# PierfrancescoArdino/C2M

Measured on AMD Instinct MI355X. Metric: generator train-step frames/sec at 128x256x7, higher is better.
Workload: dtype f32; 1 GPU; BASELINE configs[1]: 128x256, 7-frame clips (2 in + 5 predicted), batch 8/GPU, fp32, generator fwd+bwd only (no D), VGG loss on, random-init weights; global_batch=8, parallelism=single

## Files before the change

### c2m_amd/csrc/norm.hip

```cpp
#include "common.h"
#include "dtype.h"
#include <stdlib.h>

#define NORM_CHUNK 8192

struct NormShape { int N, C; long S; int mode; int chunks; };

static inline int norm_chunks(long S) { return (int)((S + NORM_CHUNK - 1) / NORM_CHUNK); }

template <class T>
__global__ __launch_bounds__(256) void norm_partial_kernel(const T* __restrict__ x, float* __restrict__ partial,
                                                            long S, int chunks) {
    __shared__ float sm[4];
    const long plane = blockIdx.x / chunks;
    const int chunk = blockIdx.x % chunks;
    const long beg = (long)chunk * NORM_CHUNK;
    const long end = beg + NORM_CHUNK < S ? beg + NORM_CHUNK : S;
    const T* __restrict__ p = x + plane * S;
    const int cnt = (int)(end - beg);
    const bool vec = (S & 3) == 0 && c2m_aligned(C2mVec4<T>::mask + 1, x);
    float s = 0.f;
    constexpr int NV = NORM_CHUNK / 1024;
    float4 keep[NV];
    if (vec) {
#pragma unroll
        for (int k = 0; k < NV; ++k) {
            const long i = beg + threadIdx.x * 4 + (long)k * 1024;
            if (i < end) {
                keep[k] = c2m_ld4(p + i);
                s += (keep[k].x + keep[k].y) + (keep[k].z + keep[k].w);
            }
        }
    } else {
        for (long i = beg + threadIdx.x; i < end; i += 256) s += c2m_ld(p, i);
    }
    s = block_sum_256(s, sm);
    const float mean = s / (float)cnt;
    float m2 = 0.f;
    if (vec) {
#pragma unroll
        for (int k = 0; k < NV; ++k) {
            const long i = beg + threadIdx.x * 4 + (long)k * 1024;
            if (i < end) {
                const float a = keep[k].x - mean, b = keep[k].y - mean, c = keep[k].z - mean, d = keep[k].w - mean;
                m2 += (a * a + b * b) + (c * c + d * d);
            }
        }
    } else {
        for (long i = beg + threadIdx.x; i < end; i += 256) { const float d = c2m_ld(p, i) - mean; m2 += d * d; }
    }
    m2 = block_sum_256(m2, sm);
    if (threadIdx.x == 0) {
        partial[(long)blockIdx.x * 2 + 0] = mean;
        partial[(long)blockIdx.x * 2 + 1] = m2;
    }
}

__global__ void norm_finalize_kernel(const float* __restrict__ partial, float* __restrict__ mean_out,
                                     float* __restrict__ invstd_out, float* __restrict__ running_mean,
                                     float* __restrict__ running_var, NormShape sh, float eps, float momentum) {
    const int nstat = sh.mode == 0 ? sh.N * sh.C : sh.C;
    const int i = blockIdx.x * blockDim.x + threadIdx.x;
    if (i >= nstat) return;
    double n = 0.0, mean = 0.0, m2 = 0.0;
    const int nrep = sh.mode == 0 ? 1 : sh.N;
    for (int r = 0; r < nrep; ++r) {
        const long plane = sh.mode == 0 ? i : (long)r * sh.C + i;
        for (int c = 0; c < sh.chunks; ++c) {
            const long beg = (long)c * NORM_CHUNK;
            const double nb = (double)((beg + NORM_CHUNK < sh.S ? beg + NORM_CHUNK : sh.S) - beg);
            const double mb = partial[(plane * sh.chunks + c) * 2 + 0];
            const double vb = partial[(plane * sh.chunks + c) * 2 + 1];
            const double tot = n + nb;
            const double delta = mb - mean;
            mean += delta * nb / tot;
            m2 += vb + delta * delta * n * nb / tot;
            n = tot;
        }
    }
    const double var = m2 / n;
    mean_out[i] = (float)mean;
    invstd_out[i] = (float)(1.0 / sqrt(var + (double)eps));
    if (running_mean) {
        const double unbiased = n > 1.0 ? m2 / (n - 1.0) : var;
        running_mean[i] = (float)((1.0 - momentum) * running_mean[i] + momentum * mean);
        running_var[i] = (float)((1.0 - momentum) * running_var[i] + momentum * unbiased);
    }
}

__global__ __launch_bounds__(256) void norm_finalize_bn_kernel(const float* __restrict__ partial,
                                                               float* __restrict__ mean_out,
                                                               float* __restrict__ invstd_out,
                                                               float* __restrict__ running_mean,
                                                               float* __restrict__ running_var, NormShape sh, float eps,
                                                               float momentum) {
    const int lane = threadIdx.x & 63;
    const int ch = blockIdx.x * 4 + (threadIdx.x >> 6);
    if (ch >= sh.C) return;
    double n = 0.0, mean = 0.0, m2 = 0.0;
    const int total = sh.N * sh.chunks;
    for (int e = lane; e < total; e += 64) {
        const int r = e / sh.chunks, c = e - r * sh.chunks;
        const long q = (((long)r * sh.C + ch) * sh.chunks + c) * 2;
        const long beg = (long)c * NORM_CHUNK;
        const double nb = (double)((beg + NORM_CHUNK < sh.S ? beg + NORM_CHUNK : sh.S) - beg);
        const double mb = partial[q], vb = partial[q + 1];
        const double tot = n + nb, delta = mb - mean;
        mean += delta * nb / tot;
        m2 += vb + delta * delta * n * nb / tot;
        n = tot;
    }
#pragma unroll
    for (int o = 32; o > 0; o >>= 1) {
        const double nb = __shfl_down(n, o, 64), mb = __shfl_down(mean, o, 64), vb = __shfl_down(m2, o, 64);
        const double tot = n + nb;
        if (tot > 0.0) {
            const double delta = mb - mean;
            mean += delta * nb / tot;
            m2 += vb + delta * delta * n * nb / tot;
            n = tot;
        }
    }
    if (lane != 0) return;
    const double var = m2 / n;
    mean_out[ch] = (float)mean;
    invstd_out[ch] = (float)(1.0 / sqrt(var + (double)eps));
    if (running_mean) {
        const double unbiased = n > 1.0 ? m2 / (n - 1.0) : var;
        running_mean[ch] = (float)((1.0 - momentum) * running_mean[ch] + momentum * mean);
        running_var[ch] = (float)((1.0 - momentum) * running_var[ch] + momentum * unbiased);
    }
}

C2M_API long c2m_norm_workspace_floats(int N, int C, long S) { return (long)N * C * norm_chunks(S) * 4; }

C2M_API int c2m_norm_stats(const void* x, float* mean, float* invstd, float* running_mean, float* running_var,
                           float* workspace, int N, int C, long S, int mode, float eps, float momentum, int dt, void* stream) {
    C2M_ENTER();
    if ((long)N * C * S <= 0) return 0;
    NormShape sh{N, C, S, mode, norm_chunks(S)};
    hipStream_t s = (hipStream_t)stream;
    C2M_DISPATCH_DT(dt, hipLaunchKernelGGL(norm_partial_kernel<T>, dim3((unsigned)((long)N * C * sh.chunks)), dim3(256), 0, s,
                                           (const T*)x, workspace, S, sh.chunks););
    const int nstat = mode == 0 ? N * C : C;
    if (mode == 1 && N * sh.chunks >= 16)
        hipLaunchKernelGGL(norm_finalize_bn_kernel, dim3(c2m_cdiv(C, 4)), dim3(256), 0, s, workspace, mean, invstd,
                           running_mean, running_var, sh, eps, momentum);
    else
        hipLaunchKernelGGL(norm_finalize_kernel, dim3(c2m_cdiv(nstat, 128)), dim3(128), 0, s, workspace, mean, invstd,
                           running_mean, running_var, sh, eps, momentum);
    return (int)hipGetLastError();
}

template <class T>
struct ApplyP {
    const T* x; const float* mean; const float* invstd; const float* gamma; const float* beta; const T* gb;
    T* y;
    int N, C; long S; int mode; int act; float slope;
};

template <class T>
__global__ void norm_apply_kernel(const ApplyP<T> p) {
    const long total = (long)p.N * p.C * p.S;
    for (long i = blockIdx.x * (long)blockDim.x + threadIdx.x; i < total; i += (long)gridDim.x * blockDim.x) {
        const long plane = i / p.S;
        const long s = i - plane * p.S;
        const int c = (int)(plane % p.C);
        const int n = (int)(plane / p.C);
        const int st = p.mode == 0 ? (int)plane : c;
        const float xhat = (c2m_ld(p.x, i) - p.mean[st]) * p.invstd[st];
        float v;
        if (p.gb) {
            const long gbase = ((long)n * 2 * p.C + c) * p.S + s;
            v = xhat * (1.0f + c2m_ld(p.gb, gbase)) + c2m_ld(p.gb, gbase + (long)p.C * p.S);
        } else if (p.gamma) {
            v = xhat * p.gamma[c] + p.beta[c];
        } else {
            v = xhat;
        }
        c2m_st(p.y, i, c2m_act(v, p.act, p.slope));
    }
}

template <class T>
// ... 158 lines not shown
    }
    m2 = block_sum_256(m2, sm);
    const double var = (double)m2 / (double)S;
    const float invstd = (float)(1.0 / sqrt(var + (double)eps));
    if (threadIdx.x == 0) { mean_out[plane] = mean; invstd_out[plane] = invstd; }
    const float ga = p.gamma ? p.gamma[c] : 1.f, be = p.gamma ? p.beta[c] : 0.f;
    T* __restrict__ y = p.y + plane * p.S;
    const T* __restrict__ g0 = p.gb ? p.gb + ((long)n * 2 * p.C + c) * p.S : nullptr;
    const T* __restrict__ g1 = p.gb ? g0 + (long)p.C * p.S : nullptr;
#pragma unroll
    for (int k = 0; k < NV; ++k) {
        const int i = threadIdx.x * 4 + k * 1024;
        if (i < S) {
            const float4 v = keep[k];
            float4 sc = make_float4(ga, ga, ga, ga), sh = make_float4(be, be, be, be);
            if (p.gb) {
                const float4 a = c2m_ld4(g0 + i);
                sc = make_float4(1.0f + a.x, 1.0f + a.y, 1.0f + a.z, 1.0f + a.w);
                sh = c2m_ld4(g1 + i);
            }
            float4 o;
            o.x = c2m_act((v.x - mean) * invstd * sc.x + sh.x, p.act, p.slope);
            o.y = c2m_act((v.y - mean) * invstd * sc.y + sh.y, p.act, p.slope);
            o.z = c2m_act((v.z - mean) * invstd * sc.z + sh.z, p.act, p.slope);
            o.w = c2m_act((v.w - mean) * invstd * sc.w + sh.w, p.act, p.slope);
            c2m_st4(y + i, o);
        }
    }
}

template <class T, int NE>
__global__ __launch_bounds__(256) void norm_bn_small_fused_kernel(const ApplyP<T> p, float* __restrict__ mean_out,
                                                                  float* __restrict__ invstd_out, float* __restrict__ running_mean,
                                                                  float* __restrict__ running_var, float eps, float momentum) {
    __shared__ float sm[4];
    const int c = blockIdx.x;
    const int S = (int)p.S, total = p.N * S;
    const long cstride = (long)p.C * p.S;
    const unsigned magic = (unsigned)((0x100000000ULL + (unsigned)S - 1) / (unsigned)S);
    const T* __restrict__ xc = p.x + (long)c * p.S;
    float keep[NE];
    float s = 0.f;
#pragma unroll
    for (int k = 0; k < NE; ++k) {
        const int e = threadIdx.x + k * 256;
        keep[k] = 0.f;
        if (e < total) {
            const int n = S == 1 ? e : (int)__umulhi((unsigned)e, magic), q = e - n * S;
            keep[k] = c2m_ld(xc, (long)n * cstride + q);
            s += keep[k];
        }
    }
    s = block_sum_256(s, sm);
    const float mean = s / (float)total;
    float m2 = 0.f;
#pragma unroll
    for (int k = 0; k < NE; ++k) {
        const int e = threadIdx.x + k * 256;
        if (e < total) { const float d = keep[k] - mean; m2 += d * d; }
    }
    m2 = block_sum_256(m2, sm);
    const double var = (double)m2 / (double)total;
    const float invstd = (float)(1.0 / sqrt(var + (double)eps));
    if (threadIdx.x == 0) {
        mean_out[c] = mean; invstd_out[c] = invstd;
        if (running_mean) {
            const double unbiased = total > 1 ? (double)m2 / (double)(total - 1) : var;
            running_mean[c] = (float)((1.0 - momentum) * running_mean[c] + momentum * (double)mean);
            running_var[c] = (float)((1.0 - momentum) * running_var[c] + momentum * unbiased);
        }
    }
    const float ga = p.gamma ? p.gamma[c] : 1.f, be = p.gamma ? p.beta[c] : 0.f;
    T* __restrict__ yc = p.y + (long)c * p.S;
#pragma unroll
    for (int k = 0; k < NE; ++k) {
        const int e = threadIdx.x + k * 256;
        if (e < total) {
            const int n = S == 1 ? e : (int)__umulhi((unsigned)e, magic), q = e - n * S;
            c2m_st(yc, (long)n * cstride + q, c2m_act((keep[k] - mean) * invstd * ga + be, p.act, p.slope));
        }
    }
}

static int norm_fused_on = [] { const char* e = getenv("C2M_NORM_FUSED"); return e ? atoi(e) & 3 : 3; }();
C2M_API int c2m_norm_set_fused(int mask) { const int old = norm_fused_on; norm_fused_on = mask & 3; return old; }

C2M_API int c2m_norm_fwd(const void* x, float* mean, float* invstd, float* running_mean, float* running_var, float* workspace,
                         const float* gamma, const float* beta, const void* gb, void* y, int N, int C, long S, int mode,
                         float eps, float momentum, int act, float slope, int dt, void* stream) {
    C2M_ENTER();
    if ((long)N * C * S <= 0) return 0;
    if ((norm_fused_on & 1) && mode == 0 && S <= 32768 && norm_vec_ok(S, x, y, gb, nullptr, dt)) {
        C2M_DISPATCH_DT(dt,
            ApplyP<T> p{(const T*)x, mean, invstd, gamma, beta, (const T*)gb, (T*)y, N, C, S, mode, act, slope};
            if (S <= 8192)
                hipLaunchKernelGGL((norm_inst_fused_kernel<T, 8>), dim3((unsigned)((long)N * C)), dim3(256), 0, (hipStream_t)stream, p, mean, invstd, eps);
            else
                hipLaunchKernelGGL((norm_inst_fused_kernel<T, 32>), dim3((unsigned)((long)N * C)), dim3(256), 0, (hipStream_t)stream, p, mean, invstd, eps););
        return (int)hipGetLastError();
    }
    if ((norm_fused_on & 2) && mode == 1 && !gb && (long)N * S <= 8192) {
        const long tot = (long)N * S;
        C2M_DISPATCH_DT(dt,
            ApplyP<T> p{(const T*)x, mean, invstd, gamma, beta, nullptr, (T*)y, N, C, S, mode, act, slope};
            if (tot <= 2048)
                hipLaunchKernelGGL((norm_bn_small_fused_kernel<T, 8>), dim3((unsigned)C), dim3(256), 0, (hipStream_t)stream, p, mean, invstd, running_mean, running_var, eps, momentum);
            else
                hipLaunchKernelGGL((norm_bn_small_fused_kernel<T, 32>), dim3((unsigned)C), dim3(256), 0, (hipStream_t)stream, p, mean, invstd, running_mean, running_var, eps, momentum););
        return (int)hipGetLastError();
    }
    const int rc = c2m_norm_stats(x, mean, invstd, running_mean, running_var, workspace, N, C, S, mode, eps, momentum, dt, stream);
    if (rc) return rc;
    return c2m_norm_apply(x, mean, invstd, gamma, beta, gb, y, nullptr, N, C, S, mode, act, slope, dt, stream);
}

template <class T>
struct BwdP {
    const T* x; const T* gy; const float* mean; const float* invstd; const float* gamma; const float* beta;
    const T* gb;
    T* ggb;
    float* partial;
    float* coef;
    float* dgamma; float* dbeta;
    T* dx;
    int N, C; long S; int mode; int act; float slope; int chunks;
};

__device__ __forceinline__ float act_grad(float pre, int act, float slope) {
    switch (act) {
        case C2M_ACT_RELU: return pre > 0.f ? 1.f : 0.f;
        case C2M_ACT_LRELU: return pre > 0.f ? 1.f : slope;
        default: return 1.f;
    }
}

template <class T>
__global__ __launch_bounds__(256) void norm_bwd_reduce_kernel(const BwdP<T> p) {
    __shared__ float sm[4];
    const long plane = blockIdx.x / p.chunks;
    const int chunk = blockIdx.x % p.chunks;
    const long beg = (long)chunk * NORM_CHUNK;
    const long end = beg + NORM_CHUNK < p.S ? beg + NORM_CHUNK : p.S;
    const int c = (int)(plane % p.C);
    const int n = (int)(plane / p.C);
    const int st = p.mode == 0 ? (int)plane : c;
    const float mean = p.mean[st], invstd = p.invstd[st];
// ... 498 lines not shown
```

### c2m_amd/modules/generator/generator.py

```python
import torch
import torch.nn as nn

from ... import ops
from ..layers.residual_block import ResidualBlock, ResidualSpadeBlock
from ..layers.same_block import SameBlock2d
from ..layers.down_block import DownBlock2d
from ..layers.up_block import UpBlock2d
from ..layers.common import conv_module
from .flowembedder import FlowEmbedder


class OcclusionAwareGenerator(nn.Module):
    def __init__(self, model_params, flow_params, input_channel, dataset):
        super().__init__()
        self.input_channel = input_channel
        self.block_expansion = model_params["block_expansion"]
        self.num_down_blocks = model_params["num_down_blocks"]
        self.max_expansion = model_params["max_expansion"]
        self.num_bottleneck_blocks = model_params["num_bottleneck_blocks"]
        self.padding_mode = model_params["padding_mode"]
        self.use_spade = model_params["use_spade"]
        self.use_skip = model_params["use_skip"]
        self.spade_params = None
        self.flow_params = flow_params
# ... 25 lines not shown
                ups.append(UpBlock2d(cin, cout, kernel_size=3, padding=1, padding_mode=pm, reshape_3d=False,
                                     input_2d=True))
        self.up_blocks = nn.ModuleList(ups)
        self.middle = nn.Sequential(*[ResidualBlock(width(nd), width(nd), kernel_size=3, padding=1)
                                      for _ in range(self.num_bottleneck_blocks)])
        self.final = nn.Sequential(nn.Conv2d(self.block_expansion, 3, kernel_size=7, padding=3), nn.Sigmoid())
        if self.use_spade:
            self.upsample = nn.Upsample(scale_factor=2, mode="bilinear")
            self.flowembedder = FlowEmbedder(self.flow_params)

    @staticmethod
    def deform_input(inp, optical_flow):
        h, w = inp.shape[2:]
        if tuple(optical_flow.shape[2:]) != (h, w):
            optical_flow = ops.resize_bilinear(optical_flow.detach(), (h, w)) if not optical_flow.requires_grad \
                else _resize_with_grad(optical_flow, (h, w))
        return ops.flow_warp(inp, optical_flow)

    def apply_optical(self, input_ref=None, optical_flow=None, occlusion_map=None):
        warped = self.deform_input(input_ref, optical_flow)
        if occlusion_map is None:
            return warped
        if warped.shape[2:] != occlusion_map.shape[2:]:
            occlusion_map = _resize_with_grad(occlusion_map, warped.shape[2:])
        return warped * occlusion_map

    def get_cond_dims(self, num_downs=0):
        num_downs = min(num_downs, self.flow_params["num_down_blocks"])
        return [min(self.max_expansion, self.block_expansion * (2 ** num_downs))]

    def get_cond_maps(self, label):
        return [[m] for m in self.flowembedder(label)]

    def forward(self, first_frame, flow, occlusion_map):
        nd = self.num_down_blocks
        if self.use_spade:
            img_warp = ops.flow_warp(first_frame, flow)
            cond = self.get_cond_maps(torch.cat([img_warp, flow, occlusion_map], dim=1))
        out = self.first(first_frame)
        for blk in self.down_blocks:
            out = blk(out)
        if not self.use_spade:
            out = self.apply_optical(input_ref=out, optical_flow=flow, occlusion_map=occlusion_map)
        for blk in self.middle:
            out = blk(out)
        if "kitti" in self.dataset:
            xw = self.first_warped(ops.flow_warp(first_frame, flow))
            for blk in self.down_blocks_warped:
                xw = blk(xw)
            occ = occlusion_map
            if xw.shape[2:] != occ.shape[2:]:
                occ = _resize_with_grad(occ, xw.shape[2:])
            out = self.pre_decode[0](torch.cat([out, xw * occ], dim=1))
        for i, blk in enumerate(self.up_blocks):
            if self.use_spade:
                c = cond[nd - i]
                if out.shape[-2:] != c[0].shape[-2:]:
                    out = ops.resize_bilinear_grad(out, c[0].shape[-2:])
                out = ops.upsample2x(blk(out, *c))
            else:
                out = blk(out)
        if out.shape[-2:] != first_frame.shape[-2:]:
            out = ops.resize_bilinear_grad(out, first_frame.shape[-2:])
        return conv_module(out, self.final[0], act="sigmoid")


def _resize_with_grad(x, size):
    return torch.nn.functional.interpolate(x, size=tuple(size), mode="bilinear")
```

### c2m_amd/modules/layers/common.py

```python
import torch

from ... import ops


def pad_triple(padding):
    if isinstance(padding, int):
        return (padding, padding, padding)
    p = list(padding)
    if len(p) == 6:
        if p[0] != p[1] or p[2] != p[3] or p[4] != p[5]:
            raise NotImplementedError("asymmetric 3-D padding")
        return (p[4], p[2], p[0])
    if len(p) == 3:
        return tuple(p)
    raise ValueError(f"padding {padding}")


def conv_module(x, conv, act=None, padding=None, padding_mode=None, dgrad_channels=None):
    pad = conv.padding if padding is None else padding
    mode = conv.padding_mode if padding_mode is None else padding_mode
    return ops.conv(x, conv.weight, conv.bias, stride=tuple(conv.stride), padding=tuple(pad) if not isinstance(pad, int) else pad,
                    padding_mode=mode, act=act, dgrad_channels=dgrad_channels)


# ... 5 lines not shown

    def __enter__(self):
        global _defer_counters
        self.prev, _defer_counters = _defer_counters, True

    def __exit__(self, *exc):
        global _defer_counters
        _defer_counters = self.prev
        if not self.prev:
            flush_batch_counters()


def flush_batch_counters():
    if not _pending_counters:
        return
    tensors = [v[0] for v in _pending_counters.values()]
    counts = [v[1] for v in _pending_counters.values()]
    _pending_counters.clear()
    by_dev = {}
    for t, c in zip(tensors, counts):
        by_dev.setdefault((t.device, t.dtype), ([], []))
        by_dev[(t.device, t.dtype)][0].append(t)
        by_dev[(t.device, t.dtype)][1].append(c)
    for ts, cs in by_dev.values():
        torch._foreach_add_(ts, cs)


def feeds_conv(conv, padding=None, padding_mode=None):
    pad = conv.padding if padding is None else padding
    mode = conv.padding_mode if padding_mode is None else padding_mode
    return ops.conv_consumer(conv.weight, tuple(conv.stride), tuple(pad) if not isinstance(pad, int) else pad, mode, conv.bias)


def batch_norm_module(x, bn, act=None, feeds=None, private_input=False):
    if bn.training:
        if not _defer_counters:
            bn.num_batches_tracked += 1
        else:
            ent = _pending_counters.get(id(bn.num_batches_tracked))
            if ent is None:
                _pending_counters[id(bn.num_batches_tracked)] = [bn.num_batches_tracked, 1]
            else:
                ent[1] += 1
        return ops.batch_norm_act(x, bn.weight, bn.bias, bn.running_mean, bn.running_var, act, bn.eps, bn.momentum, feeds,
                                  private_input)
    invstd = torch.rsqrt(bn.running_var + bn.eps)
    return ops.norm_apply_eval(x, bn.running_mean, invstd, bn.weight, bn.bias, act)


def instance_norm_module(x, inorm, act=None, feeds=None, private_input=False):
    return ops.instance_norm_act(x, inorm.weight, inorm.bias, act, inorm.eps, feeds, private_input)


def fold_time(x):
    b, c, t, h, w = x.shape
    return x.permute(2, 0, 1, 3, 4).reshape(t * b, c, h, w)


def unfold_time(x, t):
    tb, c, h, w = x.shape
    return x.reshape(t, tb // t, c, h, w).permute(1, 2, 0, 3, 4)
```

### c2m_amd/modules/layers/down_block.py

```python
from torch import nn

from .common import conv_module, batch_norm_module, pad_triple


class DownBlock2d(nn.Module):
    def __init__(self, in_features, out_features, kernel_size=(3, 3), stride=(1, 1), padding=1, padding_mode='zeros',
                 use_norm=True):
        super().__init__()
        self.conv = nn.Conv2d(in_channels=in_features, out_channels=out_features, stride=stride,
                              kernel_size=kernel_size, padding=padding, groups=1, padding_mode=padding_mode)
        self.norm = nn.BatchNorm2d(out_features, affine=True)
        self.use_norm = use_norm

    def forward(self, x):
        if not self.use_norm:
            return conv_module(x, self.conv, act="lrelu")
        return batch_norm_module(conv_module(x, self.conv), self.norm, act="lrelu", private_input=True)


class DownBlock3d(nn.Module):
    def __init__(self, in_features, out_features, kernel_size=[3, 3, 3], stride=[1, 1, 1], padding=[1, 1, 1],
                 padding_mode='zeros', use_norm=True):
        super().__init__()
        if padding_mode not in ("reflect",):
            raise NotImplementedError(f"DownBlock3d padding_mode {padding_mode}")
        self.pad_conv = nn.ReflectionPad3d(padding)
        self.conv = nn.Conv3d(in_channels=in_features, out_channels=out_features, stride=stride,
                              kernel_size=kernel_size, padding=0, groups=1, padding_mode=padding_mode)
        self.norm = nn.BatchNorm3d(out_features, affine=True)
        self.use_norm = use_norm
        self._pad3 = pad_triple(padding)

    def forward(self, x):
        if not self.use_norm:
            return conv_module(x, self.conv, act="lrelu", padding=self._pad3, padding_mode="reflect")
        y = conv_module(x, self.conv, padding=self._pad3, padding_mode="reflect")
        return batch_norm_module(y, self.norm, act="lrelu", private_input=True)
```

### c2m_amd/modules/layers/residual_block.py

```python
import torch.nn as nn

from .common import conv_module, batch_norm_module, feeds_conv
from .spade_block import SpatiallyAdaptiveNorm


class ResidualBlock(nn.Module):
    def __init__(self, in_planes, out_planes, kernel_size, padding):
        super().__init__()
        self.padding = nn.ReflectionPad2d(padding)
        self.conv1 = nn.Conv2d(in_channels=in_planes, out_channels=out_planes, kernel_size=kernel_size, padding=0)
        self.conv2 = nn.Conv2d(in_channels=out_planes, out_channels=out_planes, kernel_size=kernel_size, padding=0)
        self.norm1 = nn.BatchNorm2d(in_planes, affine=True)
        self.norm2 = nn.BatchNorm2d(out_planes, affine=True)
        self._pad = padding

    def forward(self, x):
        out = batch_norm_module(x, self.norm1, act="relu", feeds=feeds_conv(self.conv1, self._pad, "reflect"))
        out = conv_module(out, self.conv1, padding=self._pad, padding_mode="reflect")
        out = batch_norm_module(out, self.norm2, act="relu", feeds=feeds_conv(self.conv2, self._pad, "reflect"), private_input=True)
        out = conv_module(out, self.conv2, padding=self._pad, padding_mode="reflect")
        return out + x


class ResidualSpadeBlock(nn.Module):
    def __init__(self, cond_dims, in_planes, out_planes, kernel_size, padding, spade_params):
        super().__init__()
        self.cond_dims = cond_dims
        self.spade_params = spade_params
        self.padding = nn.ReflectionPad2d(padding)
        self.conv1 = nn.Conv2d(in_channels=in_planes, out_channels=out_planes, kernel_size=kernel_size, padding=0)
        self.conv2 = nn.Conv2d(in_channels=out_planes, out_channels=out_planes, kernel_size=kernel_size, padding=0)
        self.norm1 = SpatiallyAdaptiveNorm(in_planes, cond_dims)
        self.norm2 = SpatiallyAdaptiveNorm(out_planes, cond_dims)
        self.learned_shortcut = (in_planes != out_planes)
        if self.learned_shortcut:
            self.conv_s = nn.Conv2d(in_planes, out_planes, kernel_size=1, bias=False)
            self.norm_s = SpatiallyAdaptiveNorm(in_planes, cond_dims)
        self._pad = padding

    def forward(self, x, *cond_inputs):
        dx = self.norm1(x, *cond_inputs, act="lrelu", feeds=feeds_conv(self.conv1, self._pad, "reflect"))
        dx = conv_module(dx, self.conv1, padding=self._pad, padding_mode="reflect")
        dx = self.norm2(dx, *cond_inputs, act="lrelu", feeds=feeds_conv(self.conv2, self._pad, "reflect"), private_input=True)
        dx = conv_module(dx, self.conv2, padding=self._pad, padding_mode="reflect")
        if self.learned_shortcut:
            x_s = self.norm_s(x, *cond_inputs, act="lrelu", feeds=feeds_conv(self.conv_s))
            return dx + conv_module(x_s, self.conv_s)
        return dx
```

### c2m_amd/modules/model.py

```python
import functools

import numpy as np
import torch
import torch.nn as nn
import torch.optim as optim

from .. import ops
from ..optim import Adam
from ..utils import utils as U
from ..losses import losses
from .appearance_encoder.appearance_encoder import AppearanceEncoder
from .motion_estimator.dense_motion import DenseMotionNetwork
from .generator.generator import OcclusionAwareGenerator
from .discriminator import discriminator
from .layers.common import fold_time, unfold_time, deferred_batch_counters


def get_norm_layer(norm_type='instance'):
    if norm_type == 'batch':
        return functools.partial(nn.BatchNorm2d, affine=True)
    if norm_type == 'instance':
        return functools.partial(nn.InstanceNorm2d, affine=False, track_running_stats=True)
    raise NotImplementedError('normalization layer [%s] is not found' % norm_type)

# ... 70 lines not shown
        if self.train_params["loss_weights"][f"feature_matching_{dis_type}"] > 0:
            for a, b in zip(pred_real['feature_maps_%s' % 0], pred_fake['feature_maps_%s' % 0]):
                loss_fm = loss_fm + ops.l1_mean(b, a.detach())
        return loss_g_gan, loss_fm

    def _resize_inputs(self, get):
        sf = self.model_params["common_params"]["scale_factor"]
        r = U.resize_video
        return dict(frames=r(get("video"), sf, mode="bilinear"), bg_mask=r(get("bg_mask"), sf, mode="nearest"),
                    fg_mask=r(get("fg_mask"), sf, mode="nearest"),
                    instance=r(get("instance_mask").float(), sf, mode="nearest").int(),
                    input_of=r(get("input_of"), sf, mode="bilinear", is_flow=True),
                    input_occ=r(get("input_occ"), sf, mode="bilinear"))

    def _encoder_input(self, v):
        t_in = self.train_params["num_input_frames"]
        seg = torch.cat([v["bg_mask"][:, :, :t_in], v["fg_mask"][:, :, :t_in]], 1)
        parts = [_stack_time(v["frames"][:, :, :t_in]), _stack_time(seg),
                 _stack_time(v["instance"][:, :, :t_in]).to(v["frames"].dtype)]
        if v["input_of"] is not None:
            parts += [_stack_time(v["input_of"][:, :, :t_in]), _stack_time(v["input_occ"][:, :, :t_in])]
        return torch.cat(parts, 1)

    def _draw_latent(self, gnn, device):
        tp = self.train_params
        z_dim = self.model_params["motion_estimator"]["sparse_motion_estimator"]["z_dim"]
        return torch.FloatTensor(gnn.x.shape[0], tp["num_predicted_frames"], z_dim).normal_(0, 1).to(device)

    def _generate(self, v, out):
        tp = self.train_params
        t_in, T = tp["num_input_frames"], tp["num_predicted_frames"]
        last = v["frames"][:, :, t_in - 1]
        b, c, h, w = last.shape
        rep = last.unsqueeze(0).expand(T, b, c, h, w).reshape(T * b, c, h, w)
        gen = self.generator(rep, fold_time(out["dense_motion_bw"]), fold_time(out["occlusion_bw"]))
        out["generated"] = unfold_time(gen, T)
        with torch.no_grad():
            sparse = fold_time(out["sparse_motion_bw"])
            out["generated_sparse"] = unfold_time(ops.flow_warp(rep, sparse), T)
            out["generated_sparse_occ"] = unfold_time(ops.flow_warp(rep, sparse, fold_time(out["sparse_occ_bw"])), T)
        return out

    def forward(self, data_batch):
        with deferred_batch_counters():
            return self._forward(data_batch)

    def _forward(self, data_batch):
        tp = self.train_params
        t_in = tp["num_input_frames"]
        v = self._resize_inputs(data_batch.get)
        sf = self.model_params["common_params"]["scale_factor"]
        target_bw_of = U.resize_video(data_batch.get("target_bw_of"), sf, mode="bilinear", is_flow=True)
        target_bw_occ = U.resize_video(data_batch.get("target_bw_occ"), sf, mode="bilinear")
        target_fw_of = U.resize_video(data_batch.get("target_fw_of"), sf, mode="bilinear", is_flow=True)
        target_fw_occ = U.resize_video(data_batch.get("target_fw_occ"), sf, mode="bilinear")
        pl = getattr(self.objective_func, "perceptual_loss", None)
        if pl is not None:
            pl.prefetch(v["frames"][:, :, t_in:])
        gnn = data_batch["tracking_gnn"]
        rng = data_batch.get("rng") or {}
        latent = rng["latent_traj"] if "latent_traj" in rng else self._draw_latent(gnn, gnn.x.device)
        app = self.appearance_encoder({"first_frame": self._encoder_input(v), "tracking_gnn": gnn})
        motion_input = dict(frames=v["frames"], bg_mask=v["bg_mask"], fg_mask=v["fg_mask"], instance=v["instance"],
                            input_of=v["input_of"], input_occ=v["input_occ"], target_bw_of=target_bw_of,
                            target_bw_occ=target_bw_occ, target_fw_of=target_fw_of, target_fw_occ=target_fw_occ,
                            tracking_gnn=gnn, latent=latent, eps=rng.get("eps"), click_index=rng.get("click_index"))
        out = {}
        out.update(self.motion_encoder(app, motion_input))
        out = self._generate(v, out)
        ops.aux_join(*[t for k, t in out.items() if k.startswith("theta_")], *(pl.prefetched_tensors() if pl is not None else []))
# ... 34 lines not shown
```

### c2m_amd/ops.py

```python
import collections
import ctypes
import os
import weakref
import math

import numpy as np
import torch

from . import _lib

G, WG = _lib.GEOM, _lib.WINO_GEOM

ACT = {None: 0, "none": 0, "relu": 1, "lrelu": 2, "sigmoid": 3}
LRELU_SLOPE = 0.2


def _stream():
    return ctypes.c_void_p(_raw_stream(_cur_device()))


_raw_stream = getattr(torch._C, "_cuda_getCurrentRawStream", None)
_cur_device = getattr(torch._C, "_cuda_getDevice", None)
if _raw_stream is None or _cur_device is None:
    _raw_stream = lambda idx: torch.cuda.current_stream(idx).cuda_stream
# ... 1717 lines not shown
        raise ValueError(f"conv_transpose2d: inconsistent geometry {tuple(x.shape)} vs {pl.out_shape}")
    with torch.no_grad():
        y = _conv_dgrad(pl, w, x, True, x.dtype)
        if b is not None or ACT[act]:
            y = _as(y, torch.float32)
            _lib.check(_lib.lib().c2m_bias_act(_p(y), _p(b), N, Co, Ho * Wo, ACT[act], float(slope), _stream()), "bias_act")
    return y


_MAX_TENSOR_BYTES = int(0.9 * 2 ** 31)


def _chunks_for_2gib(xs, ws, stride, pad):
    n, cin, cout = xs[0], xs[1], ws[0]
    sp_in = [d for d in xs[2:]]
    k3 = list(ws[2:])
    nd = len(sp_in)
    padded, out = 1, 1
    for d in range(nd):
        padded *= sp_in[d] + 2 * pad[3 - nd + d]
        out *= max((sp_in[d] + 2 * pad[3 - nd + d] - k3[d]) // stride[3 - nd + d] + 1, 1)
    per_image = 4 * max(cin * padded, cout * out)
    if n * per_image < _MAX_TENSOR_BYTES:
        return 1
    fit = (_MAX_TENSOR_BYTES - 1) // per_image
    if fit < 1:
        raise ValueError("tensor too large: one image exceeds the 32-bit byte offsets of the gather (< 2 GiB)")
    return _cdiv(n, fit)


class _NormActFn(torch.autograd.Function):

    @staticmethod
    def forward(ctx, x, gamma, beta, gb, running_mean, running_var, mode, act, eps, momentum, feeds=None, private_input=False):
        _dev(x, gamma, beta, gb)
        x = _f(x)
        ctx.gb_dtype = gb.dtype if gb is not None else None
        gb = _as(gb, x.dtype)
        dt = _dt(x)
        N, C = x.shape[0], x.shape[1]
        S = x.numel() // (N * C)
        for name, t, want in (("gamma", gamma, C), ("beta", beta, C), ("running_mean", running_mean, C), ("running_var", running_var, C),
                              ("SPADE map", gb, 2 * x.numel())):
            if t is not None and t.numel() != want:
                raise RuntimeError(f"norm: {name} has {t.numel()} elements, expected {want} for an input of shape {tuple(x.shape)}")
        L = _lib.lib()
        nstat = N * C if mode == 0 else C
        mean = torch.empty(nstat, device=x.device, dtype=torch.float32)
        invstd = torch.empty_like(mean)
        ws = torch.empty(L.c2m_norm_workspace_floats(N, C, S), device=x.device, dtype=torch.float32)
        y = torch.empty_like(x)
        ctx.nc8 = bool(_NC8 and _NC8_NORM and dt == 1 and x.dim() == 4 and S % 8 == 0 and C >= 16 and x.shape[3] >= 16 and S >= 512)
        only = False
        if feeds is not None and dt == 1 and S % 8 == 0:
            only = _consumer_reads_only_nc8(x, feeds)
        yn = torch.empty((N, _cdiv(C, 8)) + tuple(x.shape[2:]) + (8,), device=x.device, dtype=BF16) if (ctx.nc8 or only) else None
        if yn is None:
            _lib.check(L.c2m_norm_fwd(_p(x), _p(mean), _p(invstd), _p(running_mean), _p(running_var), _p(ws), _p(gamma), _p(beta), _p(gb),
                                      _p(y), N, C, S, mode, eps, momentum, ACT[act], LRELU_SLOPE, dt, _stream()), "norm_fwd")
        else:
            _lib.check(L.c2m_norm_stats(_p(x), _p(mean), _p(invstd), _p(running_mean), _p(running_var), _p(ws), N, C, S, mode,
                                        eps, momentum, dt, _stream()), "norm_stats")
            _lib.check(L.c2m_norm_apply(_p(x), _p(mean), _p(invstd), _p(gamma), _p(beta), _p(gb), None if only else _p(y), _p(yn), N, C, S,
                                        mode, ACT[act], LRELU_SLOPE, dt, _stream()), "norm_apply")
        if only and _NC8_POISON:
            y.fill_(float("nan"))
        _NormActFn.last_only = only
        ctx.cfg = (N, C, S, mode, act)
        ctx.dx_nc8_only = bool(private_input and _NC8_GRAD and dt == 1 and S % 8 == 0 and getattr(x, "_c2m_bwd_nc8", False))
        ctx.save_for_backward(x, gamma, beta, gb, mean, invstd)
        if yn is None:
            return y, None
        ctx.mark_non_differentiable(yn)
        return y, yn

    @staticmethod
    def backward(ctx, gy, _gyn=None):
        x, gamma, beta, gb, mean, invstd = ctx.saved_tensors
        N, C, S, mode, act = ctx.cfg
        L = _lib.lib()
        gy = _as(gy, x.dtype)
        only = ctx.dx_nc8_only
        dx = torch.empty_like(x)
        dxn = torch.empty((N, _cdiv(C, 8)) + tuple(x.shape[2:]) + (8,), device=x.device, dtype=BF16) if (ctx.nc8 or only) else None
        ggb = torch.empty_like(gb) if gb is not None else None
        dgamma = torch.empty_like(gamma) if gamma is not None else None
        dbeta = torch.empty_like(beta) if gamma is not None else None
        ws = torch.empty(L.c2m_norm_workspace_floats(N, C, S), device=x.device, dtype=torch.float32)
        _lib.check(L.c2m_norm_bwd(_p(x), _p(gy), _p(mean), _p(invstd), _p(gamma), _p(beta), _p(gb), _p(ggb), _p(dgamma),
                                  _p(dbeta), None if only else _p(dx), _p(dxn), _p(ws), N, C, S, mode, ACT[act], LRELU_SLOPE, _dt(x),
                                  _stream()),
                   "norm_bwd")
        if only and _NC8_POISON:
            dx.fill_(float("nan"))
        if dxn is not None and only:
            _mark_nc8_only(dx, dxn)
        elif dxn is not None:
            dx._c2m_nc8 = (dx._version, dxn)
        if ggb is not None and ggb.dtype != ctx.gb_dtype:
            ggb = ggb.to(ctx.gb_dtype)
        return dx, dgamma, dbeta, ggb, None, None, None, None, None, None, None, None


def _norm_act(*args):
    y, yn = _NormActFn.apply(*args)
    if yn is not None and _NormActFn.last_only:
        _mark_nc8_only(y, yn)
    elif yn is not None:
        y._c2m_nc8 = (y._version, yn)
    return y


def batch_norm_act(x, gamma, beta, running_mean, running_var, act=None, eps=1e-5, momentum=0.1, feeds=None, private_input=False):
    return _norm_act(x, gamma, beta, None, running_mean, running_var, 1, act, eps, momentum, feeds, private_input)


def instance_norm_act(x, gamma=None, beta=None, act=None, eps=1e-5, feeds=None, private_input=False):
    return _norm_act(x, gamma, beta, None, None, None, 0, act, eps, 0.1, feeds, private_input)


def spade_norm_act(x, gamma_beta, act=None, eps=1e-5, feeds=None, private_input=False):
    return _norm_act(x, None, None, gamma_beta, None, None, 0, act, eps, 0.1, feeds, private_input)


class _FlowWarpFn(torch.autograd.Function):
    @staticmethod
    def forward(ctx, img, flow, occ):
        _dev(img, flow, occ)
        ctx.flow_dtype = flow.dtype
        img, flow = _f(img), _as(flow, torch.float32)
        occ = _as(occ, torch.float32)
        N, C, H, W = img.shape
        assert flow.shape == (N, 2, H, W), f"flow {tuple(flow.shape)} vs image {tuple(img.shape)}"
        assert occ is None or occ.shape == (N, 1, H, W)
        out = torch.empty_like(img)
        _lib.check(_lib.lib().c2m_flow_warp_fwd(_p(img), _p(flow), _p(occ), _p(out), N, C, H, W, _dt(img), _stream()),
                   "flow_warp")
        ctx.save_for_backward(img, flow, occ)
        return out

    @staticmethod
    def backward(ctx, gout):
        img, flow, occ = ctx.saved_tensors
        N, C, H, W = img.shape
        L = _lib.lib()
        gimg = torch.empty_like(img) if ctx.needs_input_grad[0] else None
        gflow = torch.empty_like(flow) if ctx.needs_input_grad[1] else None
# ... 1306 lines not shown
```

### include/c2m_hip.h

```cpp
#ifndef C2M_HIP_H
#define C2M_HIP_H
#include <stdint.h>
#ifdef __cplusplus
extern "C" {
#endif

enum { C2M_ACT_NONE = 0, C2M_ACT_RELU = 1, C2M_ACT_LRELU = 2, C2M_ACT_SIGMOID = 3 };

#include "c2m_geom.h"
int c2m_abi_version(void);
int c2m_geom_len(void);
int c2m_wino_geom_len(void);

int c2m_conv_igemm_splits(int M, int nk, int Npix);
int c2m_conv_igemm(const float* A, const void* X, void* Y, void* Y_interior, const float* bias, const int* ktab,
                   const int64_t* geom, int act, float slope, void* stream);
int c2m_splitk_reduce(const float* slab, void* out, const float* bias, long total, int splits, long chan_stride,
                      int M, int act, float slope, int dt , void* stream);

int c2m_conv_wgrad_splits(int M, int J, int Npix);
int c2m_conv_wgrad_rows(int M, int ngroups);
int c2m_conv_wgrad(const void* dY, const void* X, float* slab, float* dW, float* db, const int* jtab,
                   const int64_t* geom, void* stream);

// ... 33 lines not shown
                  const int64_t* geom, int act, float slope, void* stream);

long c2m_wino4_upack_floats(int M, int K);
int c2m_wino4_filter_transform(const float* w, float* upack, int Cout, int Cin, int dgrad, void* stream);
int c2m_wino4_regions(int Ho, int Wo);
int c2m_conv_wino4(const float* upack, const float* X, float* Y, float* Y_interior, const float* bias,
                   const int64_t* geom, int act, float slope, void* stream);

int c2m_wino_wgrad_splits(int M, int K, int nimg, int H, int W);
int c2m_conv_wino_wgrad(const float* dY, const float* X, float* slab, float* dbslab, float* dW, float* db, int M, int K,
                        int nimg, int H, int W, int reflect, void* stream);
int c2m_conv_wino_wgrad3d(const float* dY, const float* X, float* slab, float* dbslab, float* dW, float* db,
                          int M, int Cin, int N, int T, int H, int W, int reflect, void* stream);

long c2m_ring_pack_floats(int C, int M);
int c2m_ring_pack(const float* w, float* apack, int C, int M, void* stream);
int c2m_reflect_ring_dgrad(const float* apack, const float* w, const float* dY, float* dX, int N, int C, int M, int H, int W,
                           void* stream);
int c2m_reflect_ring_buffer(const float* apack, const float* dY, float* R, int N, int C, int M, int H, int W, int r_l,
                            void* stream);

int c2m_reflect_border_add(const void* dXpad, void* dX, long NC, int T, int H, int W, int pt, int ph, int pw,
                           int dt, void* stream);
int c2m_reflect_fold(const void* dXpad, void* dX, long NC, int T, int H, int W, int pt, int ph, int pw,
                     int dt, void* stream);

long c2m_norm_workspace_floats(int N, int C, long S);
int c2m_norm_stats(const void* x, float* mean, float* invstd, float* running_mean, float* running_var,
                   float* workspace, int N, int C, long S, int mode, float eps, float momentum, int dt, void* stream);
int c2m_norm_set_fused(int on);
int c2m_norm_fwd(const void* x, float* mean, float* invstd, float* running_mean, float* running_var, float* workspace,
                 const float* gamma, const float* beta, const void* gb, void* y, int N, int C, long S, int mode, float eps,
                 float momentum, int act, float slope, int dt, void* stream);
int c2m_norm_apply(const void* x, const float* mean, const float* invstd, const float* gamma, const float* beta,
                   const void* gb, void* y, void* y_nc8, int N, int C, long S, int mode, int act, float slope, int dt, void* stream);
int c2m_norm_bwd(const void* x, const void* gy, const float* mean, const float* invstd, const float* gamma,
                 const float* beta, const void* gb, void* ggb, float* dgamma, float* dbeta, void* dx, void* dx_nc8,
                 float* workspace, int N, int C, long S, int mode, int act, float slope, int dt, void* stream);
int c2m_act_bwd(const void* y, const void* gy, void* gx, long total, int act, float slope, int dt, void* stream);
int c2m_grad_to_nc8(int mode, const void* y, const void* t, const void* gy, const float* gl, void* g_nc8, long N, int C, long S,
                    long count, int act, float slope, void* stream);

int c2m_flow_warp_fwd(const void* img, const float* flow, const float* occ, void* out, int N, int C, int H, int W,
                      int dt, void* stream);
long c2m_flow_warp_bwd_workspace_bytes(int N, int C, int H, int W, int want_gimg, int want_gflow);
int c2m_flow_warp_bwd(const void* img, const float* flow, const float* occ, const void* gout, void* gimg,
                      float* gflow, int N, int C, int H, int W, void* workspace, int dt, void* stream);
int c2m_resize_bilinear(const void* in, void* out, long NC, int Hi, int Wi, int Ho, int Wo, int align,
                        double scale_factor, int dt, void* stream);
int c2m_resize_bilinear_bwd(const void* gout, void* gin, long NC, int Hi, int Wi, int Ho, int Wo, int align, int dt,
                            void* stream);
int c2m_upsample2x_fwd(const void* in, void* out, long NC, int Hi, int Wi, int dt, void* stream);
int c2m_upsample2x_nc8(const void* in_nc8, void* out_nc8, long NCB, int Hi, int Wi, void* stream);
int c2m_upsample2x_bwd(const void* gout, void* gin, long NC, int Hi, int Wi, int dt, void* stream);
int c2m_roi_align_fwd(const float* feat, const float* boxes, float* out, int K, int C, int H, int W, int PH, int PW,
                      float spatial_scale, void* stream);
int c2m_roi_align_bwd(const float* boxes, const float* gout, float* gfeat, int N, int K, int C, int H, int W, int PH,
                      int PW, float spatial_scale, void* stream);
int c2m_maxpool2x2_fwd(const void* in, void* out, long NC, int Hi, int Wi, int dt, void* stream);
int c2m_maxpool2x2_bwd(const void* in, const void* gout, void* gin, long NC, int Hi, int Wi, int dt, void* stream);
int c2m_maxpool2x2_relu_bwd(const void* in, const void* gout, void* gin, long NC, int Hi, int Wi, int dt, void* stream);

int c2m_resample2d_fwd(const float* img, const float* flow, float* out, int N, int C, int H, int W, void* stream);
int c2m_channelnorm_fwd(const float* x, float* out, int N, int C, int H, int W, void* stream);
int c2m_correlation_out_size(int H, int pad, int kernel_size, int max_displacement, int stride1);
int c2m_correlation_fwd(const float* in1, const float* in2, float* out, int N, int C, int H, int W, int pad,
// ... 124 lines not shown
```

Before: 902.2 frames/s.

## Run generator encoder once per source frame instead of per repeated copy

The generator previously received the last input frame tiled T times and ran the first conv, down blocks (and, for SPADE, middle blocks) on identical copies. Now it runs those layers on the B unique frames and expands to T*B only where the flow-dependent path begins. BatchNorm statistics are unchanged because the batch is just repeated, and a replication count passed to the norm kernels keeps the unbiased running-variance update equal to that of the repeated batch. This cuts encoder forward and backward work by roughly a factor of T, at the cost of extra API plumbing and an expand/reshape copy.

After: 970.2 frames/s, median of 6. 1.08x the previous value.

```diff
diff --git a/c2m_amd/csrc/norm.hip b/c2m_amd/csrc/norm.hip
--- a/c2m_amd/csrc/norm.hip
+++ b/c2m_amd/csrc/norm.hip
@@ -56,9 +56,15 @@
     }
 }
 
+__device__ inline double norm_unbiased_var(double m2, double n, double var, int rep) {
+    const double nr = n * (double)rep;
+    return nr > 1.0 ? m2 * (double)rep / (nr - 1.0) : var;
+}
+
 __global__ void norm_finalize_kernel(const float* __restrict__ partial, float* __restrict__ mean_out,
                                      float* __restrict__ invstd_out, float* __restrict__ running_mean,
-                                     float* __restrict__ running_var, NormShape sh, float eps, float momentum) {
+                                     float* __restrict__ running_var, NormShape sh, float eps, float momentum,
+                                     int rep) {
     const int nstat = sh.mode == 0 ? sh.N * sh.C : sh.C;
     const int i = blockIdx.x * blockDim.x + threadIdx.x;
     if (i >= nstat) return;
@@ -82,7 +88,7 @@
     mean_out[i] = (float)mean;
     invstd_out[i] = (float)(1.0 / sqrt(var + (double)eps));
     if (running_mean) {
-        const double unbiased = n > 1.0 ? m2 / (n - 1.0) : var;
+        const double unbiased = norm_unbiased_var(m2, n, var, rep);
         running_mean[i] = (float)((1.0 - momentum) * running_mean[i] + momentum * mean);
         running_var[i] = (float)((1.0 - momentum) * running_var[i] + momentum * unbiased);
     }
@@ -93,7 +99,7 @@
                                                                float* __restrict__ invstd_out,
                                                                float* __restrict__ running_mean,
                                                                float* __restrict__ running_var, NormShape sh, float eps,
-                                                               float momentum) {
+                                                               float momentum, int rep) {
     const int lane = threadIdx.x & 63;
     const int ch = blockIdx.x * 4 + (threadIdx.x >> 6);
     if (ch >= sh.C) return;
@@ -126,7 +132,7 @@
     mean_out[ch] = (float)mean;
     invstd_out[ch] = (float)(1.0 / sqrt(var + (double)eps));
     if (running_mean) {
-        const double unbiased = n > 1.0 ? m2 / (n - 1.0) : var;
+        const double unbiased = norm_unbiased_var(m2, n, var, rep);
         running_mean[ch] = (float)((1.0 - momentum) * running_mean[ch] + momentum * mean);
         running_var[ch] = (float)((1.0 - momentum) * running_var[ch] + momentum * unbiased);
     }
@@ -134,10 +140,12 @@
 
 C2M_API long c2m_norm_workspace_floats(int N, int C, long S) { return (long)N * C * norm_chunks(S) * 4; }
 
-C2M_API int c2m_norm_stats(const void* x, float* mean, float* invstd, float* running_mean, float* running_var,
-                           float* workspace, int N, int C, long S, int mode, float eps, float momentum, int dt, void* stream) {
+C2M_API int c2m_norm_stats_rep(const void* x, float* mean, float* invstd, float* running_mean, float* running_var,
+                               float* workspace, int N, int C, long S, int mode, float eps, float momentum, int rep, int dt,
+                               void* stream) {
     C2M_ENTER();
     if ((long)N * C * S <= 0) return 0;
+    if (rep < 1 || (mode == 0 && rep != 1)) return (int)hipErrorInvalidValue;
     NormShape sh{N, C, S, mode, norm_chunks(S)};
     hipStream_t s = (hipStream_t)stream;
     C2M_DISPATCH_DT(dt, hipLaunchKernelGGL(norm_partial_kernel<T>, dim3((unsigned)((long)N * C * sh.chunks)), dim3(256), 0, s,
@@ -145,11 +153,16 @@
     const int nstat = mode == 0 ? N * C : C;
     if (mode == 1 && N * sh.chunks >= 16)
         hipLaunchKernelGGL(norm_finalize_bn_kernel, dim3(c2m_cdiv(C, 4)), dim3(256), 0, s, workspace, mean, invstd,
-                           running_mean, running_var, sh, eps, momentum);
+                           running_mean, running_var, sh, eps, momentum, rep);
     else
         hipLaunchKernelGGL(norm_finalize_kernel, dim3(c2m_cdiv(nstat, 128)), dim3(128), 0, s, workspace, mean, invstd,
-                           running_mean, running_var, sh, eps, momentum);
+                           running_mean, running_var, sh, eps, momentum, rep);
     return (int)hipGetLastError();
+}
+
+C2M_API int c2m_norm_stats(const void* x, float* mean, float* invstd, float* running_mean, float* running_var,
+                           float* workspace, int N, int C, long S, int mode, float eps, float momentum, int dt, void* stream) {
+    return c2m_norm_stats_rep(x, mean, invstd, running_mean, running_var, workspace, N, C, S, mode, eps, momentum, 1, dt, stream);
 }
 
 template <class T>
@@ -374,7 +387,8 @@
 template <class T, int NE>
 __global__ __launch_bounds__(256) void norm_bn_small_fused_kernel(const ApplyP<T> p, float* __restrict__ mean_out,
                                                                   float* __restrict__ invstd_out, float* __restrict__ running_mean,
-                                                                  float* __restrict__ running_var, float eps, float momentum) {
+                                                                  float* __restrict__ running_var, float eps, float momentum,
+                                                                  int rep) {
     __shared__ float sm[4];
     const int c = blockIdx.x;
     const int S = (int)p.S, total = p.N * S;
@@ -407,7 +421,7 @@
     if (threadIdx.x == 0) {
         mean_out[c] = mean; invstd_out[c] = invstd;
         if (running_mean) {
-            const double unbiased = total > 1 ? (double)m2 / (double)(total - 1) : var;
+            const double unbiased = norm_unbiased_var((double)m2, (double)total, var, rep);
             running_mean[c] = (float)((1.0 - momentum) * running_mean[c] + momentum * (double)mean);
             running_var[c] = (float)((1.0 - momentum) * running_var[c] + momentum * unbiased);
         }
@@ -427,11 +441,12 @@
 static int norm_fused_on = [] { const char* e = getenv("C2M_NORM_FUSED"); return e ? atoi(e) & 3 : 3; }();
 C2M_API int c2m_norm_set_fused(int mask) { const int old = norm_fused_on; norm_fused_on = mask & 3; return old; }
 
-C2M_API int c2m_norm_fwd(const void* x, float* mean, float* invstd, float* running_mean, float* running_var, float* workspace,
-                         const float* gamma, const float* beta, const void* gb, void* y, int N, int C, long S, int mode,
-                         float eps, float momentum, int act, float slope, int dt, void* stream) {
+C2M_API int c2m_norm_fwd_rep(const void* x, float* mean, float* invstd, float* running_mean, float* running_var, float* workspace,
+                             const float* gamma, const float* beta, const void* gb, void* y, int N, int C, long S, int mode,
+                             float eps, float momentum, int rep, int act, float slope, int dt, void* stream) {
     C2M_ENTER();
     if ((long)N * C * S <= 0) return 0;
+    if (rep < 1 || (mode == 0 && rep != 1)) return (int)hipErrorInvalidValue;
     if ((norm_fused_on & 1) && mode == 0 && S <= 32768 && norm_vec_ok(S, x, y, gb, nullptr, dt)) {
         C2M_DISPATCH_DT(dt,
             ApplyP<T> p{(const T*)x, mean, invstd, gamma, beta, (const T*)gb, (T*)y, N, C, S, mode, act, slope};
@@ -446,14 +461,21 @@
         C2M_DISPATCH_DT(dt,
             ApplyP<T> p{(const T*)x, mean, invstd, gamma, beta, nullptr, (T*)y, N, C, S, mode, act, slope};
             if (tot <= 2048)
-                hipLaunchKernelGGL((norm_bn_small_fused_kernel<T, 8>), dim3((unsigned)C), dim3(256), 0, (hipStream_t)stream, p, mean, invstd, running_mean, running_var, eps, momentum);
+                hipLaunchKernelGGL((norm_bn_small_fused_kernel<T, 8>), dim3((unsigned)C), dim3(256), 0, (hipStream_t)stream, p, mean, invstd, running_mean, running_var, eps, momentum, rep);
             else
-                hipLaunchKernelGGL((norm_bn_small_fused_kernel<T, 32>), dim3((unsigned)C), dim3(256), 0, (hipStream_t)stream, p, mean, invstd, running_mean, running_var, eps, momentum););
+                hipLaunchKernelGGL((norm_bn_small_fused_kernel<T, 32>), dim3((unsigned)C), dim3(256), 0, (hipStream_t)stream, p, mean, invstd, running_mean, running_var, eps, momentum, rep););
         return (int)hipGetLastError();
     }
-    const int rc = c2m_norm_stats(x, mean, invstd, running_mean, running_var, workspace, N, C, S, mode, eps, momentum, dt, stream);
+    const int rc = c2m_norm_stats_rep(x, mean, invstd, running_mean, running_var, workspace, N, C, S, mode, eps, momentum, rep, dt, stream);
     if (rc) return rc;
     return c2m_norm_apply(x, mean, invstd, gamma, beta, gb, y, nullptr, N, C, S, mode, act, slope, dt, stream);
+}
+
+C2M_API int c2m_norm_fwd(const void* x, float* mean, float* invstd, float* running_mean, float* running_var, float* workspace,
+                         const float* gamma, const float* beta, const void* gb, void* y, int N, int C, long S, int mode,
+                         float eps, float momentum, int act, float slope, int dt, void* stream) {
+    return c2m_norm_fwd_rep(x, mean, invstd, running_mean, running_var, workspace, gamma, beta, gb, y, N, C, S, mode, eps, momentum, 1,
+                            act, slope, dt, stream);
 }
 
 template <class T>
diff --git a/c2m_amd/modules/generator/generator.py b/c2m_amd/modules/generator/generator.py
--- a/c2m_amd/modules/generator/generator.py
+++ b/c2m_amd/modules/generator/generator.py
@@ -81,20 +81,27 @@
     def get_cond_maps(self, label):
         return [[m] for m in self.flowembedder(label)]
 
-    def forward(self, first_frame, flow, occlusion_map):
-        nd = self.num_down_blocks
+    def forward(self, first_frame, flow, occlusion_map, source_repeats=1):
+        nd, T = self.num_down_blocks, int(source_repeats)
+        if T < 1 or flow.shape[0] != T * first_frame.shape[0]:
+            raise ValueError(f"generator: {first_frame.shape[0]} source frames x {T} repeats vs {flow.shape[0]} flow frames")
+        frames = first_frame if T == 1 else _repeat_frames(first_frame, T)
         if self.use_spade:
-            img_warp = ops.flow_warp(first_frame, flow)
+            img_warp = ops.flow_warp(frames, flow)
             cond = self.get_cond_maps(torch.cat([img_warp, flow, occlusion_map], dim=1))
         out = self.first(first_frame)
         for blk in self.down_blocks:
-            out = blk(out)
+            out = blk(out, rep=T)
         if not self.use_spade:
+            if T != 1:
+                out = _repeat_frames(out, T)
             out = self.apply_optical(input_ref=out, optical_flow=flow, occlusion_map=occlusion_map)
         for blk in self.middle:
-            out = blk(out)
+            out = blk(out, rep=T if self.use_spade else 1)
+        if self.use_spade and T != 1:
+            out = _repeat_frames(out, T)
         if "kitti" in self.dataset:
-            xw = self.first_warped(ops.flow_warp(first_frame, flow))
+            xw = self.first_warped(ops.flow_warp(frames, flow))
             for blk in self.down_blocks_warped:
                 xw = blk(xw)
             occ = occlusion_map
@@ -114,5 +121,9 @@
         return conv_module(out, self.final[0], act="sigmoid")
 
 
+def _repeat_frames(x, t):
+    return x.unsqueeze(0).expand(t, *x.shape).reshape(t * x.shape[0], *x.shape[1:])
+
+
 def _resize_with_grad(x, size):
     return torch.nn.functional.interpolate(x, size=tuple(size), mode="bilinear")
diff --git a/c2m_amd/modules/layers/common.py b/c2m_amd/modules/layers/common.py
--- a/c2m_amd/modules/layers/common.py
+++ b/c2m_amd/modules/layers/common.py
@@ -61,7 +61,7 @@
     return ops.conv_consumer(conv.weight, tuple(conv.stride), tuple(pad) if not isinstance(pad, int) else pad, mode, conv.bias)
 
 
-def batch_norm_module(x, bn, act=None, feeds=None, private_input=False):
+def batch_norm_module(x, bn, act=None, feeds=None, private_input=False, rep=1):
     if bn.training:
         if not _defer_counters:
             bn.num_batches_tracked += 1
@@ -72,7 +72,7 @@
             else:
                 ent[1] += 1
         return ops.batch_norm_act(x, bn.weight, bn.bias, bn.running_mean, bn.running_var, act, bn.eps, bn.momentum, feeds,
-                                  private_input)
+                                  private_input, rep)
     invstd = torch.rsqrt(bn.running_var + bn.eps)
     return ops.norm_apply_eval(x, bn.running_mean, invstd, bn.weight, bn.bias, act)
 
diff --git a/c2m_amd/modules/layers/down_block.py b/c2m_amd/modules/layers/down_block.py
--- a/c2m_amd/modules/layers/down_block.py
+++ b/c2m_amd/modules/layers/down_block.py
@@ -12,10 +12,10 @@
         self.norm = nn.BatchNorm2d(out_features, affine=True)
         self.use_norm = use_norm
 
-    def forward(self, x):
+    def forward(self, x, rep=1):
         if not self.use_norm:
             return conv_module(x, self.conv, act="lrelu")
-        return batch_norm_module(conv_module(x, self.conv), self.norm, act="lrelu", private_input=True)
+        return batch_norm_module(conv_module(x, self.conv), self.norm, act="lrelu", private_input=True, rep=rep)
 
 
 class DownBlock3d(nn.Module):
diff --git a/c2m_amd/modules/layers/residual_block.py b/c2m_amd/modules/layers/residual_block.py
--- a/c2m_amd/modules/layers/residual_block.py
+++ b/c2m_amd/modules/layers/residual_block.py
@@ -14,10 +14,11 @@
         self.norm2 = nn.BatchNorm2d(out_planes, affine=True)
         self._pad = padding
 
-    def forward(self, x):
-        out = batch_norm_module(x, self.norm1, act="relu", feeds=feeds_conv(self.conv1, self._pad, "reflect"))
+    def forward(self, x, rep=1):
+        out = batch_norm_module(x, self.norm1, act="relu", feeds=feeds_conv(self.conv1, self._pad, "reflect"), rep=rep)
         out = conv_module(out, self.conv1, padding=self._pad, padding_mode="reflect")
-        out = batch_norm_module(out, self.norm2, act="relu", feeds=feeds_conv(self.conv2, self._pad, "reflect"), private_input=True)
+        out = batch_norm_module(out, self.norm2, act="relu", feeds=feeds_conv(self.conv2, self._pad, "reflect"), private_input=True,
+                                rep=rep)
         out = conv_module(out, self.conv2, padding=self._pad, padding_mode="reflect")
         return out + x
 
diff --git a/c2m_amd/modules/model.py b/c2m_amd/modules/model.py
--- a/c2m_amd/modules/model.py
+++ b/c2m_amd/modules/model.py
@@ -126,10 +126,10 @@
         t_in, T = tp["num_input_frames"], tp["num_predicted_frames"]
         last = v["frames"][:, :, t_in - 1]
         b, c, h, w = last.shape
-        rep = last.unsqueeze(0).expand(T, b, c, h, w).reshape(T * b, c, h, w)
-        gen = self.generator(rep, fold_time(out["dense_motion_bw"]), fold_time(out["occlusion_bw"]))
+        gen = self.generator(last, fold_time(out["dense_motion_bw"]), fold_time(out["occlusion_bw"]), source_repeats=T)
         out["generated"] = unfold_time(gen, T)
         with torch.no_grad():
+            rep = last.unsqueeze(0).expand(T, b, c, h, w).reshape(T * b, c, h, w)
             sparse = fold_time(out["sparse_motion_bw"])
             out["generated_sparse"] = unfold_time(ops.flow_warp(rep, sparse), T)
             out["generated_sparse_occ"] = unfold_time(ops.flow_warp(rep, sparse, fold_time(out["sparse_occ_bw"])), T)
diff --git a/c2m_amd/ops.py b/c2m_amd/ops.py
--- a/c2m_amd/ops.py
+++ b/c2m_amd/ops.py
@@ -1773,8 +1773,11 @@
 class _NormActFn(torch.autograd.Function):
 
     @staticmethod
-    def forward(ctx, x, gamma, beta, gb, running_mean, running_var, mode, act, eps, momentum, feeds=None, private_input=False):
+    def forward(ctx, x, gamma, beta, gb, running_mean, running_var, mode, act, eps, momentum, feeds=None, private_input=False, rep=1):
         _dev(x, gamma, beta, gb)
+        rep = int(rep)
+        if rep < 1 or (rep != 1 and mode != 1):
+            raise ValueError(f"norm: replication count {rep} (batch statistics only, >= 1)")
         x = _f(x)
         ctx.gb_dtype = gb.dtype if gb is not None else None
         gb = _as(gb, x.dtype)
@@ -1797,11 +1800,11 @@
             only = _consumer_reads_only_nc8(x, feeds)
         yn = torch.empty((N, _cdiv(C, 8)) + tuple(x.shape[2:]) + (8,), device=x.device, dtype=BF16) if (ctx.nc8 or only) else None
         if yn is None:
-            _lib.check(L.c2m_norm_fwd(_p(x), _p(mean), _p(invstd), _p(running_mean), _p(running_var), _p(ws), _p(gamma), _p(beta), _p(gb),
-                                      _p(y), N, C, S, mode, eps, momentum, ACT[act], LRELU_SLOPE, dt, _stream()), "norm_fwd")
+            _lib.check(L.c2m_norm_fwd_rep(_p(x), _p(mean), _p(invstd), _p(running_mean), _p(running_var), _p(ws), _p(gamma), _p(beta), _p(gb),
+                                          _p(y), N, C, S, mode, eps, momentum, rep, ACT[act], LRELU_SLOPE, dt, _stream()), "norm_fwd")
         else:
-            _lib.check(L.c2m_norm_stats(_p(x), _p(mean), _p(invstd), _p(running_mean), _p(running_var), _p(ws), N, C, S, mode,
-                                        eps, momentum, dt, _stream()), "norm_stats")
+            _lib.check(L.c2m_norm_stats_rep(_p(x), _p(mean), _p(invstd), _p(running_mean), _p(running_var), _p(ws), N, C, S, mode,
+                                            eps, momentum, rep, dt, _stream()), "norm_stats")
             _lib.check(L.c2m_norm_apply(_p(x), _p(mean), _p(invstd), _p(gamma), _p(beta), _p(gb), None if only else _p(y), _p(yn), N, C, S,
                                         mode, ACT[act], LRELU_SLOPE, dt, _stream()), "norm_apply")
         if only and _NC8_POISON:
@@ -1840,11 +1843,11 @@
             dx._c2m_nc8 = (dx._version, dxn)
         if ggb is not None and ggb.dtype != ctx.gb_dtype:
             ggb = ggb.to(ctx.gb_dtype)
-        return dx, dgamma, dbeta, ggb, None, None, None, None, None, None, None, None
-
-
-def _norm_act(*args):
-    y, yn = _NormActFn.apply(*args)
+        return dx, dgamma, dbeta, ggb, None, None, None, None, None, None, None, None, None
+
+
+def _norm_act(*args, rep=1):
+    y, yn = _NormActFn.apply(*args, rep)
     if yn is not None and _NormActFn.last_only:
         _mark_nc8_only(y, yn)
     elif yn is not None:
@@ -1852,8 +1855,8 @@
     return y
 
 
-def batch_norm_act(x, gamma, beta, running_mean, running_var, act=None, eps=1e-5, momentum=0.1, feeds=None, private_input=False):
-    return _norm_act(x, gamma, beta, None, running_mean, running_var, 1, act, eps, momentum, feeds, private_input)
+def batch_norm_act(x, gamma, beta, running_mean, running_var, act=None, eps=1e-5, momentum=0.1, feeds=None, private_input=False, rep=1):
+    return _norm_act(x, gamma, beta, None, running_mean, running_var, 1, act, eps, momentum, feeds, private_input, rep=rep)
 
 
 def instance_norm_act(x, gamma=None, beta=None, act=None, eps=1e-5, feeds=None, private_input=False):
diff --git a/include/c2m_hip.h b/include/c2m_hip.h
--- a/include/c2m_hip.h
+++ b/include/c2m_hip.h
@@ -89,6 +89,11 @@
 int c2m_norm_fwd(const void* x, float* mean, float* invstd, float* running_mean, float* running_var, float* workspace,
                  const float* gamma, const float* beta, const void* gb, void* y, int N, int C, long S, int mode, float eps,
                  float momentum, int act, float slope, int dt, void* stream);
+int c2m_norm_stats_rep(const void* x, float* mean, float* invstd, float* running_mean, float* running_var,
+                       float* workspace, int N, int C, long S, int mode, float eps, float momentum, int rep, int dt, void* stream);
+int c2m_norm_fwd_rep(const void* x, float* mean, float* invstd, float* running_mean, float* running_var, float* workspace,
+                     const float* gamma, const float* beta, const void* gb, void* y, int N, int C, long S, int mode, float eps,
+                     float momentum, int rep, int act, float slope, int dt, void* stream);
 int c2m_norm_apply(const void* x, const float* mean, const float* invstd, const float* gamma, const float* beta,
                    const void* gb, void* y, void* y_nc8, int N, int C, long S, int mode, int act, float slope, int dt, void* stream);
 int c2m_norm_bwd(const void* x, const void* gy, const float* mean, const float* invstd, const float* gamma,
```
